# lambdaclass/ethrex

Measured on NVIDIA H100. Metric: bn254_g1_msm_points_per_sec, higher is better.
Workload: dtype u32x8 Montgomery (254-bit modular integer)

## Files before the change

ethrex_b200/csrc/msm.cu:

```cuda
#include "common.cuh"
#include "tma.cuh"
#include <cstdlib>

namespace b200zk {

static constexpr int kMaxWindows = 64;
static constexpr uint32_t kMaxPipelineChunks = 64;
static constexpr int kChunk = 16;
static constexpr int kG2MinBlocks = 1;

struct MsmPlan {
  uint32_t c, W, B;
  uint32_t chunk, T;
  uint32_t merged;
  uint32_t Wr;
  uint32_t table_stride;
  uint32_t adaptive;
};

uint32_t precompute_window(size_t n) {
  uint32_t lg = 0;
  while (((size_t)1 << lg) < n) ++lg;
  if (lg >= 20) return 20;
  if (lg <= 6) return 6;
// ... 16 lines not shown
  const uint32_t want_chunk = chunk_knob > 0 ? (uint32_t)chunk_knob : (uint32_t)kChunk;
  p.chunk = p.B < want_chunk ? p.B : want_chunk;
  p.T = p.B / p.chunk;
  p.merged = 0; p.Wr = p.W; p.table_stride = 0;
  static int adaptive = -1;
  if (adaptive < 0) { const char* e = getenv("B200ZK_SORT_MATCH"); adaptive = (e && *e == '1') ? 0 : 1; }
  p.adaptive = (uint32_t)adaptive;
  return p;
}

B2_D void decode_scalar(uint4 lo, uint4 hi, uint32_t flags, uint32_t s[8]) {
  if (flags & B200ZK_SCALARS_BE) {
    s[7] = __byte_perm(lo.x, 0, 0x0123); s[6] = __byte_perm(lo.y, 0, 0x0123); s[5] = __byte_perm(lo.z, 0, 0x0123); s[4] = __byte_perm(lo.w, 0, 0x0123);
    s[3] = __byte_perm(hi.x, 0, 0x0123); s[2] = __byte_perm(hi.y, 0, 0x0123); s[1] = __byte_perm(hi.z, 0, 0x0123); s[0] = __byte_perm(hi.w, 0, 0x0123);
  } else {
    s[0] = lo.x; s[1] = lo.y; s[2] = lo.z; s[3] = lo.w; s[4] = hi.x; s[5] = hi.y; s[6] = hi.z; s[7] = hi.w;
  }
  Fr f;
#pragma unroll
  for (int k = 0; k < 8; ++k) f.v[k] = s[k];
  if (flags & B200ZK_SCALARS_RAW) {
  } else if (flags & B200ZK_SCALARS_MONT) {
#pragma unroll 1
    for (int k = 0; k < 5; ++k) {
      Fr m = Fr::modulus(), t; uint32_t borrow = detail::sub8(t.v, f.v, m.v);
      if (!borrow) f = t;
    }
    f = Fr::from_mont(f);
  } else if (f.v[7] >= FrCfg::mod(7)) {
#pragma unroll 1
    for (int k = 0; k < 5; ++k) {
      Fr m = Fr::modulus(), t; uint32_t borrow = detail::sub8(t.v, f.v, m.v);
      if (!borrow) f = t;
    }
  }
#pragma unroll
  for (int k = 0; k < 8; ++k) s[k] = f.v[k];
}

B2_D uint32_t window_bits(const uint32_t s[8], uint32_t w, uint32_t c) {
  uint32_t bit = w * c;
  uint32_t limb = bit >> 5, off = bit & 31;
  if (limb >= 8) return 0;
  uint64_t v = s[limb];
  if (limb + 1 < 8) v |= (uint64_t)s[limb + 1] << 32;
  return (uint32_t)(v >> off) & ((1u << c) - 1u);
}

static constexpr uint32_t kNoDigit = 0xffffffffu;

static constexpr uint32_t kSkewLanes = 3;
B2_D uint32_t warp_group(uint32_t key, bool active, uint32_t* rank, uint32_t* group_mask, bool adaptive) {
  if (adaptive) {
    const uint32_t full = __activemask();
    const uint32_t act = __ballot_sync(full, active);
    const uint32_t k0 = __shfl_sync(full, key, act ? __ffs(act) - 1 : 0);
    const uint32_t m0 = __ballot_sync(full, active && key == k0);
    if (__popc(m0) < kSkewLanes) {
      *rank = 0;
      *group_mask = 1u << (threadIdx.x & 31);
      return 1;
    }
  }
  uint32_t mask = __match_any_sync(__activemask(), active ? key : kNoDigit);
  uint32_t lane = threadIdx.x & 31;
  *rank = __popc(mask & ((1u << lane) - 1u));
  *group_mask = mask;
  return __popc(mask);
}

static constexpr uint32_t kHistTile = 256;
__global__ void __launch_bounds__(kHistTile) msm_hist(const void* scalars, size_t n, uint32_t flags, MsmPlan pl, uint32_t* hist, uint32_t* digits) {
  __shared__ __align__(128) uint4 tile[2][kHistTile * 2];
  __shared__ uint64_t bar[2];
  const size_t tiles = (n + kHistTile - 1) / kHistTile;
  if (threadIdx.x == 0) { tma::barrier_init(&bar[0], 1); tma::barrier_init(&bar[1], 1); tma::barrier_init_fence(); }
  __syncthreads();
  auto issue = [&](size_t tl, uint32_t buf) {
    size_t first = tl * kHistTile;
    uint32_t bytes = (uint32_t)((n - first < kHistTile ? n - first : kHistTile) * 32);
    tma::barrier_expect(&bar[buf], bytes);
    tma::bulk_load(tile[buf], reinterpret_cast<const uint8_t*>(scalars) + first * 32, bytes, &bar[buf]);
  };
  if (threadIdx.x == 0 && blockIdx.x < tiles) issue(blockIdx.x, 0);
  uint32_t it = 0;
  for (size_t tl = blockIdx.x; tl < tiles; tl += gridDim.x, ++it) {
    const uint32_t buf = it & 1;
    if (threadIdx.x == 0 && tl + gridDim.x < tiles) issue(tl + gridDim.x, buf ^ 1);
    tma::barrier_wait(&bar[buf], (it >> 1) & 1);
    const size_t i = tl * kHistTile + threadIdx.x;
    const bool live = i < n;
    uint32_t s[8] = {0, 0, 0, 0, 0, 0, 0, 0};
    if (live) decode_scalar(tile[buf][2 * threadIdx.x], tile[buf][2 * threadIdx.x + 1], flags, s);
    uint32_t carry = 0;
    for (uint32_t w = 0; w < pl.W; ++w) {
      uint32_t coef = window_bits(s, w, pl.c) + carry;
      carry = 0;
      uint32_t neg = 0, mag = coef;
      if (w + 1 < pl.W && coef >= pl.B) { carry = 1; neg = 0x80000000u; mag = (1u << pl.c) - coef; }
      uint32_t code = mag ? ((mag - 1) | neg) : kNoDigit;
      if (live) digits[(size_t)w * n + i] = code;
      uint32_t rank, gm;
      uint32_t cnt = warp_group(mag - 1, live && mag != 0, &rank, &gm, pl.adaptive != 0);
      if (live && mag && rank == 0) atomicAdd(&hist[(pl.merged ? 0 : (size_t)w * pl.B) + (mag - 1)], cnt);
    }
    __syncthreads();
  }
}

static constexpr int kScatterIlp = 4;
__global__ void __launch_bounds__(256) msm_scatter(const uint32_t* __restrict__ digits, size_t n, MsmPlan pl, uint32_t* cursor, uint32_t* idx) {
  const size_t total = (size_t)pl.W * n;
  const size_t stride = (size_t)gridDim.x * blockDim.x;
  const size_t total_pad = (total + 31) & ~(size_t)31;
  for (size_t t0 = blockIdx.x * (size_t)blockDim.x + threadIdx.x; t0 < total_pad; t0 += stride * kScatterIlp) {
    uint32_t code[kScatterIlp], g[kScatterIlp], rank[kScatterIlp], mask[kScatterIlp], base[kScatterIlp];
    size_t w[kScatterIlp];
    bool live[kScatterIlp], active[kScatterIlp];
#pragma unroll
    for (int u = 0; u < kScatterIlp; ++u) {
      const size_t t = t0 + u * stride;
      live[u] = t < total_pad;
      code[u] = (live[u] && t < total) ? __ldg(digits + t) : kNoDigit;
      active[u] = code[u] != kNoDigit;
      w[u] = live[u] ? t / n : 0;
      g[u] = (pl.merged ? 0u : (uint32_t)(w[u] * pl.B)) + (code[u] & 0x7fffffffu);
    }
#pragma unroll
    for (int u = 0; u < kScatterIlp; ++u) {
      base[u] = 0; rank[u] = 0; mask[u] = 0;
      if (live[u]) {
        uint32_t cnt = warp_group(g[u], active[u], &rank[u], &mask[u], pl.adaptive != 0);
        if (active[u] && rank[u] == 0) base[u] = atomicAdd(&cursor[g[u]], cnt);
      }
    }
#pragma unroll
    for (int u = 0; u < kScatterIlp; ++u) {
      if (live[u]) {
        uint32_t bs = __shfl_sync(mask[u], base[u], __ffs(mask[u]) - 1);
        const size_t t = t0 + u * stride;
        if (active[u]) idx[bs + rank[u]] = (uint32_t)((t - w[u] * n) + (pl.merged ? w[u] * pl.table_stride : 0)) | (code[u] & 0x80000000u);
      }
    }
  }
}

static constexpr uint32_t kSortTile = 1024;
static constexpr uint32_t kSortMaxW = 16;
static constexpr uint32_t kSortMaxBins = 1024;
static constexpr uint32_t kSortMaxFine = 2048;
static constexpr uint32_t kSortCountSub = 4;
static constexpr int kFineIlp = 8;

struct SortPlan {
  uint32_t fb;
  uint32_t C;
  uint32_t NC;
  uint32_t range;
  uint32_t G;
};
static bool make_sort_plan(size_t n, const MsmPlan& pl, int sm_count, SortPlan* sp) {
  const size_t G = (size_t)pl.Wr * pl.B;
  uint32_t kb = 0;
  while (((size_t)1 << kb) < G) ++kb;
  if (pl.W > kSortMaxW || kb < 12 || n < ((size_t)1 << 16)) return false;
  uint32_t cb = kb > 19 ? 10 : 9;
  if (kb - cb > 11) return false;
  sp->fb = kb - cb;
  sp->C = (uint32_t)((G + ((size_t)1 << sp->fb) - 1) >> sp->fb);
  sp->G = (uint32_t)G;
  uint32_t nc = (uint32_t)sm_count;
  size_t tiles = (n + kSortTile - 1) / kSortTile;
  if (nc > tiles) nc = (uint32_t)tiles;
  size_t per = ((tiles + nc - 1) / nc) * kSortTile;
  sp->NC = (uint32_t)((n + per - 1) / per);
  sp->range = (uint32_t)per;
  return true;
}

B2_D void recode_scalar(const uint32_t s[8], const MsmPlan& pl, uint32_t (&code)[kSortMaxW]) {
  uint32_t carry = 0;
#pragma unroll
  for (uint32_t w = 0; w < kSortMaxW; ++w) {
    code[w] = kNoDigit;
    if (w < pl.W) {
      uint32_t coef = window_bits(s, w, pl.c) + carry;
      carry = 0;
      uint32_t neg = 0, mag = coef;
      if (w + 1 < pl.W && coef >= pl.B) { carry = 1; neg = 0x80000000u; mag = (1u << pl.c) - coef; }
      code[w] = mag ? ((mag - 1) | neg) : kNoDigit;
    }
  }
}

__global__ void __launch_bounds__(kHistTile) msm_sort_count(const void* scalars, size_t n, uint32_t flags, MsmPlan pl, SortPlan sp, uint32_t* cnt) {
  __shared__ __align__(128) uint4 tile[2][kHistTile * 2];
  __shared__ uint64_t bar[2];
  __shared__ uint32_t sh[kSortMaxBins];
  const uint32_t r = blockIdx.x / kSortCountSub, sub = blockIdx.x % kSortCountSub;
  for (uint32_t b = threadIdx.x; b < sp.C; b += kHistTile) sh[b] = 0;
  const size_t lo = (size_t)r * sp.range, hi = lo + sp.range < n ? lo + sp.range : n;
  const size_t tiles_all = lo < hi ? (hi - lo + kHistTile - 1) / kHistTile : 0;
  const size_t per = (tiles_all + kSortCountSub - 1) / kSortCountSub;
  const size_t t0 = sub * per, t1 = t0 + per < tiles_all ? t0 + per : tiles_all;
  if (threadIdx.x == 0) { tma::barrier_init(&bar[0], 1); tma::barrier_init(&bar[1], 1); tma::barrier_init_fence(); }
  __syncthreads();
  auto issue = [&](size_t tl, uint32_t buf) {
    size_t first = lo + tl * kHistTile;
    uint32_t bytes = (uint32_t)((hi - first < kHistTile ? hi - first : kHistTile) * 32);
    tma::barrier_expect(&bar[buf], bytes);
    tma::bulk_load(tile[buf], reinterpret_cast<const uint8_t*>(scalars) + first * 32, bytes, &bar[buf]);
  };
  if (threadIdx.x == 0 && t0 < t1) issue(t0, 0);
  uint32_t it = 0;
  for (size_t tl = t0; tl < t1; ++tl, ++it) {
    const uint32_t buf = it & 1;
    if (threadIdx.x == 0 && tl + 1 < t1) issue(tl + 1, buf ^ 1);
    tma::barrier_wait(&bar[buf], (it >> 1) & 1);
    const size_t i = lo + tl * kHistTile + threadIdx.x;
    if (i < hi) {
      uint32_t s[8], code[kSortMaxW];
      decode_scalar(tile[buf][2 * threadIdx.x], tile[buf][2 * threadIdx.x + 1], flags, s);
      recode_scalar(s, pl, code);
#pragma unroll
      for (uint32_t w = 0; w < kSortMaxW; ++w)
        if (code[w] != kNoDigit) {
          const uint32_t g = (pl.merged ? 0u : w * pl.B) + (code[w] & 0x7fffffffu);
          atomicAdd(&sh[g >> sp.fb], 1u);
        }
    }
    __syncthreads();
  }
  __syncthreads();
  for (uint32_t b = threadIdx.x; b < sp.C; b += kHistTile) if (sh[b]) atomicAdd(&cnt[(size_t)b * sp.NC + r], sh[b]);
}

struct SortCoarseSmem {
  uint2 ent[kSortTile * kSortMaxW];
  uint32_t dst[kSortTile * kSortMaxW];
  uint32_t run_base[kSortMaxBins], tile_cnt[kSortMaxBins], tile_start[kSortMaxBins];
  uint32_t warp_tot[kSortTile / 32];
  uint32_t total;
};
__global__ void __launch_bounds__(kSortTile, 1) msm_sort_coarse(const void* __restrict__ scalars, size_t n, uint32_t flags, MsmPlan pl, SortPlan sp, const uint32_t* __restrict__ base,
                                                               uint2* __restrict__ ent1) {
  extern __shared__ __align__(16) uint8_t smem_raw[];
  SortCoarseSmem& sm = *reinterpret_cast<SortCoarseSmem*>(smem_raw);
  const uint32_t r = blockIdx.x, tid = threadIdx.x;
  const size_t lo = (size_t)r * sp.range, hi = lo + sp.range < n ? lo + sp.range : n;
  const uint32_t fmask = (1u << sp.fb) - 1u;
  for (uint32_t b = tid; b < sp.C; b += kSortTile) { sm.run_base[b] = __ldg(base + (size_t)b * sp.NC + r); sm.tile_cnt[b] = 0; }
  __syncthreads();
  const uint4* sc = reinterpret_cast<const uint4*>(scalars);
  for (size_t t0 = lo; t0 < hi; t0 += kSortTile) {
    const size_t i = t0 + tid;
    uint32_t code[kSortMaxW], rank[kSortMaxW];
    const bool live = i < hi;
#pragma unroll
    for (uint32_t w = 0; w < kSortMaxW; ++w) { code[w] = kNoDigit; rank[w] = 0; }
    if (live) {
      uint32_t s[8];
      decode_scalar(__ldg(sc + 2 * i), __ldg(sc + 2 * i + 1), flags, s);
      recode_scalar(s, pl, code);
#pragma unroll
      for (uint32_t w = 0; w < kSortMaxW; ++w)
        if (code[w] != kNoDigit) {
          const uint32_t g = (pl.merged ? 0u : w * pl.B) + (code[w] & 0x7fffffffu);
          rank[w] = atomicAdd(&sm.tile_cnt[g >> sp.fb], 1u);
        }
    }
    __syncthreads();
    {
      const uint32_t v = tid < sp.C ? sm.tile_cnt[tid] : 0;
      uint32_t incl = v;
#pragma unroll
      for (int o = 1; o < 32; o <<= 1) { uint32_t t = __shfl_up_sync(0xffffffffu, incl, o); if ((tid & 31) >= (unsigned)o) incl += t; }
      if ((tid & 31) == 31) sm.warp_tot[tid >> 5] = incl;
      __syncthreads();
      uint32_t wb = 0;
      for (uint32_t k = 0; k < (tid >> 5); ++k) wb += sm.warp_tot[k];
      if (tid < sp.C) sm.tile_start[tid] = wb + incl - v;
      if (tid == kSortTile - 1) sm.total = wb + incl;
    }
    __syncthreads();
    if (live) {
#pragma unroll
      for (uint32_t w = 0; w < kSortMaxW; ++w)
        if (code[w] != kNoDigit) {
          const uint32_t g = (pl.merged ? 0u : w * pl.B) + (code[w] & 0x7fffffffu);
          const uint32_t b = g >> sp.fb, pos = sm.tile_start[b] + rank[w];
          sm.ent[pos] = make_uint2((uint32_t)(i + (pl.merged ? (size_t)w * pl.table_stride : 0)) | (code[w] & 0x80000000u), g & fmask);
          sm.dst[pos] = sm.run_base[b] + rank[w];
        }
    }
    __syncthreads();
    const uint32_t total = sm.total;
    for (uint32_t t = tid; t < total; t += kSortTile) ent1[sm.dst[t]] = sm.ent[t];
    __syncthreads();
    if (tid < sp.C) { sm.run_base[tid] += sm.tile_cnt[tid]; sm.tile_cnt[tid] = 0; }
    __syncthreads();
  }
}

static constexpr uint32_t kFineTile = 8192;
static constexpr uint32_t kFineSeg = 4 * kFineTile;
struct SortFineSmem {
  uint32_t val[kFineTile], dst[kFineTile];
  uint32_t cur[kSortMaxFine], tcnt[kSortMaxFine], tstart[kSortMaxFine];
  uint32_t warp_tot[32];
  uint32_t total;
};
B2_D void scan_fine_keys(const uint32_t* in, uint32_t* out, uint32_t F, uint32_t* warp_tot, uint32_t* total) {
  const uint32_t tid = threadIdx.x, k0 = 2 * tid, k1 = 2 * tid + 1;
  const uint32_t v0 = k0 < F ? in[k0] : 0, v1 = k1 < F ? in[k1] : 0;
  uint32_t incl = v0 + v1;
#pragma unroll
  for (int o = 1; o < 32; o <<= 1) { uint32_t t = __shfl_up_sync(0xffffffffu, incl, o); if ((tid & 31) >= (unsigned)o) incl += t; }
  if ((tid & 31) == 31) warp_tot[tid >> 5] = incl;
  __syncthreads();
  uint32_t wb = 0;
  for (uint32_t k = 0; k < (tid >> 5); ++k) wb += warp_tot[k];
  const uint32_t ex = wb + incl - v0 - v1;
  if (k0 < F) out[k0] = ex;
  if (k1 < F) out[k1] = ex + v0;
  if (tid == 1023) *total = wb + incl;
  __syncthreads();
}
__global__ void __launch_bounds__(1024) msm_sort_items(const uint32_t* __restrict__ base, SortPlan sp, uint32_t* __restrict__ item_start) {
  __shared__ uint32_t wt[32];
  const uint32_t tid = threadIdx.x;
  uint32_t v = 0;
  if (tid < sp.C) { const uint32_t sz = __ldg(base + (size_t)(tid + 1) * sp.NC) - __ldg(base + (size_t)tid * sp.NC); v = (sz + kFineSeg - 1) / kFineSeg; }
  uint32_t incl = v;
#pragma unroll
  for (int o = 1; o < 32; o <<= 1) { uint32_t t = __shfl_up_sync(0xffffffffu, incl, o); if ((tid & 31) >= (unsigned)o) incl += t; }
  if ((tid & 31) == 31) wt[tid >> 5] = incl;
  __syncthreads();
  uint32_t wb = 0;
  for (uint32_t k = 0; k < (tid >> 5); ++k) wb += wt[k];
  if (tid < sp.C) item_start[tid] = wb + incl - v;
  if (tid == sp.C - 1) item_start[sp.C] = wb + incl;
}
B2_D uint32_t item_bin(const uint32_t* __restrict__ item_start, uint32_t C, uint32_t i) {
  uint32_t lo = 0, hi = C;
  while (hi - lo > 1) { uint32_t mid = (lo + hi) >> 1; if (__ldg(item_start + mid) <= i) lo = mid; else hi = mid; }
  return lo;
}
__global__ void __launch_bounds__(1024, 2) msm_sort_fine_count(const uint2* __restrict__ ent1, SortPlan sp, const uint32_t* __restrict__ base, const uint32_t* __restrict__ item_start,
                                                               uint32_t* __restrict__ cnt2) {
  __shared__ uint32_t fh[kSortMaxFine];
  const uint32_t i = blockIdx.x, tid = threadIdx.x, F = 1u << sp.fb;
  if (i >= __ldg(item_start + sp.C)) return;
  const uint32_t b = item_bin(item_start, sp.C, i);
  const uint32_t bs = __ldg(base + (size_t)b * sp.NC), be = __ldg(base + (size_t)(b + 1) * sp.NC);
  const uint32_t s0 = bs + (i - __ldg(item_start + b)) * kFineSeg, s1 = (be - s0 > kFineSeg) ? s0 + kFineSeg : be;
  for (uint32_t k = tid; k < F; k += 1024) fh[k] = 0;
  __syncthreads();
  for (uint32_t e0 = s0 + tid; e0 < s1; e0 += 1024 * kFineIlp) {
    uint32_t kk[kFineIlp];
#pragma unroll
    for (int u = 0; u < kFineIlp; ++u) { const uint32_t e = e0 + u * 1024; kk[u] = e < s1 ? __ldg(&ent1[e].y) : 0xffffffffu; }
#pragma unroll
    for (int u = 0; u < kFineIlp; ++u) if (kk[u] != 0xffffffffu) atomicAdd(&fh[kk[u]], 1u);
  }
  __syncthreads();
  for (uint32_t k = tid; k < F; k += 1024) cnt2[(size_t)i * F + k] = fh[k];
}
__global__ void __launch_bounds__(256) msm_sort_fine_prefix(SortPlan sp, const uint32_t* __restrict__ item_start, uint32_t* __restrict__ cnt2, uint32_t* __restrict__ hist) {
  const uint32_t F = 1u << sp.fb;
  const size_t t = blockIdx.x * (size_t)blockDim.x + threadIdx.x;
  if (t >= (size_t)sp.C * F) return;
  const uint32_t b = (uint32_t)(t >> sp.fb), k = (uint32_t)t & (F - 1);
  const uint32_t i0 = __ldg(item_start + b), i1 = __ldg(item_start + b + 1);
  uint32_t run = 0;
  for (uint32_t i = i0; i < i1; ++i) {
    const size_t at = (size_t)i * F + k;
    const uint32_t c = cnt2[at];
    cnt2[at] = run;
    run += c;
  }
  if (t < sp.G) hist[t] = run;
}
__global__ void __launch_bounds__(1024, 1) msm_sort_fine_place(const uint2* __restrict__ ent1, SortPlan sp, const uint32_t* __restrict__ base, const uint32_t* __restrict__ item_start,
                                                               const uint32_t* __restrict__ cnt2, const uint32_t* __restrict__ offsets, uint32_t* __restrict__ idx) {
  extern __shared__ __align__(16) uint8_t smem_raw[];
  SortFineSmem& sm = *reinterpret_cast<SortFineSmem*>(smem_raw);
  const uint32_t i = blockIdx.x, tid = threadIdx.x, F = 1u << sp.fb;
  if (i >= __ldg(item_start + sp.C)) return;
  const uint32_t b = item_bin(item_start, sp.C, i);
  const uint32_t bs = __ldg(base + (size_t)b * sp.NC), be = __ldg(base + (size_t)(b + 1) * sp.NC);
  const uint32_t s0 = bs + (i - __ldg(item_start + b)) * kFineSeg, s1 = (be - s0 > kFineSeg) ? s0 + kFineSeg : be;
  for (uint32_t k = tid; k < F; k += 1024) {
    const size_t g = (size_t)b * F + k;
    sm.cur[k] = (g < sp.G ? __ldg(offsets + g) : 0u) + __ldg(cnt2 + (size_t)i * F + k);
    sm.tcnt[k] = 0;
  }
  __syncthreads();
  for (uint32_t t0 = s0; t0 < s1; t0 += kFineTile) {
    uint2 ev[kFineTile / 1024];
    uint32_t rank[kFineTile / 1024];
#pragma unroll
    for (int u = 0; u < (int)(kFineTile / 1024); ++u) {
      const uint32_t e = t0 + u * 1024 + tid;
      ev[u] = e < s1 ? __ldg(ent1 + e) : make_uint2(0u, 0xffffffffu);
    }
#pragma unroll
    for (int u = 0; u < (int)(kFineTile / 1024); ++u) rank[u] = ev[u].y != 0xffffffffu ? atomicAdd(&sm.tcnt[ev[u].y], 1u) : 0u;
    __syncthreads();
    scan_fine_keys(sm.tcnt, sm.tstart, F, sm.warp_tot, &sm.total);
#pragma unroll
    for (int u = 0; u < (int)(kFineTile / 1024); ++u)
      if (ev[u].y != 0xffffffffu) {
        const uint32_t pos = sm.tstart[ev[u].y] + rank[u];
        sm.val[pos] = ev[u].x;
        sm.dst[pos] = sm.cur[ev[u].y] + rank[u];
      }
    __syncthreads();
    const uint32_t total = sm.total;
    for (uint32_t t = tid; t < total; t += 1024) idx[sm.dst[t]] = sm.val[t];
    __syncthreads();
    for (uint32_t k = tid; k < F; k += 1024) { sm.cur[k] += sm.tcnt[k]; sm.tcnt[k] = 0; }
    __syncthreads();
  }
}

static constexpr int kScanThreads = 256, kScanItems = 8, kScanTile = kScanThreads * kScanItems;

B2_D uint32_t scan_value(const uint32_t* in, const uint32_t* aux, size_t i, uint32_t seg, uint32_t shift) {
  uint32_t v = in[i];
  if (!seg) return (v + (1u << shift) - 1u) >> shift;
  return (v != 0 && (aux[i] % seg) != 0) ? 1u : 0u;
}

__global__ void __launch_bounds__(kScanThreads) scan_tile_sums(const uint32_t* in, const uint32_t* aux, size_t G, uint32_t seg, uint32_t shift, uint32_t* tile_sums) {
  __shared__ uint32_t red[kScanThreads / 32];
  size_t base = (size_t)blockIdx.x * kScanTile + (size_t)threadIdx.x * kScanItems;
  uint32_t s = 0;
#pragma unroll
  for (int k = 0; k < kScanItems; ++k) if (base + k < G) s += scan_value(in, aux, base + k, seg, shift);
#pragma unroll
  for (int o = 16; o; o >>= 1) s += __shfl_xor_sync(0xffffffffu, s, o);
  if ((threadIdx.x & 31) == 0) red[threadIdx.x >> 5] = s;
  __syncthreads();
  if (threadIdx.x == 0) {
    uint32_t t = 0;
    for (int k = 0; k < kScanThreads / 32; ++k) t += red[k];
    tile_sums[blockIdx.x] = t;
  }
}
__global__ void __launch_bounds__(1024) scan_tile_offsets(uint32_t* tile_sums, size_t tiles) {
  __shared__ uint32_t buf[1024];
  __shared__ uint32_t carry;
  if (threadIdx.x == 0) carry = 0;
  __syncthreads();
  for (size_t base = 0; base < tiles; base += 1024) {
    size_t i = base + threadIdx.x;
    uint32_t v = i < tiles ? tile_sums[i] : 0;
    buf[threadIdx.x] = v;
    __syncthreads();
    for (int o = 1; o < 1024; o <<= 1) {
      uint32_t t = threadIdx.x >= (unsigned)o ? buf[threadIdx.x - o] : 0;
      __syncthreads();
      buf[threadIdx.x] += t;
      __syncthreads();
    }
    uint32_t incl = buf[threadIdx.x], c0 = carry;
    __syncthreads();
    if (i < tiles) tile_sums[i] = c0 + incl - v;
    if (threadIdx.x == 1023) carry = c0 + incl;
    __syncthreads();
  }
}
__global__ void __launch_bounds__(kScanThreads) scan_apply(const uint32_t* in, const uint32_t* aux, size_t G, uint32_t seg, uint32_t shift, const uint32_t* tile_offsets, uint32_t* offsets, uint32_t* cursor) {
  __shared__ uint32_t warp_tot[kScanThreads / 32];
  size_t base = (size_t)blockIdx.x * kScanTile + (size_t)threadIdx.x * kScanItems;
  uint32_t v[kScanItems], s = 0;
#pragma unroll
  for (int k = 0; k < kScanItems; ++k) { v[k] = base + k < G ? scan_value(in, aux, base + k, seg, shift) : 0; s += v[k]; }
  uint32_t incl = s;
#pragma unroll
  for (int o = 1; o < 32; o <<= 1) { uint32_t t = __shfl_up_sync(0xffffffffu, incl, o); if ((threadIdx.x & 31) >= (unsigned)o) incl += t; }
  if ((threadIdx.x & 31) == 31) warp_tot[threadIdx.x >> 5] = incl;
  __syncthreads();
  uint32_t wbase = 0;
  for (unsigned k = 0; k < (threadIdx.x >> 5); ++k) wbase += warp_tot[k];
  uint32_t run = tile_offsets[blockIdx.x] + wbase + incl - s;
#pragma unroll
  for (int k = 0; k < kScanItems; ++k) {
    if (base + k < G) { offsets[base + k] = seg ? run + (aux[base + k] + seg - 1) / seg : run; if (cursor) cursor[base + k] = run; }
    run += v[k];
  }
  if (blockIdx.x == gridDim.x - 1 && threadIdx.x == kScanThreads - 1) offsets[G] = seg ? run + (aux[G] + seg - 1) / seg : run;
}

static constexpr uint32_t kSegLenMax = 256;
static constexpr uint32_t kTreeRadix = 64;
static constexpr uint32_t kDirectRuns = 4;

static uint32_t pick_slice_len(size_t M, size_t resident) {
  if (M == 0) return kSegLenMax;
  size_t per_thread = (M + resident - 1) / resident;
  size_t waves = (per_thread + kSegLenMax - 1) / kSegLenMax;
  size_t len = (M + resident * waves - 1) / (resident * waves);
  if (len < 16) len = 16;
  if (len > kSegLenMax) len = kSegLenMax;
  return (uint32_t)len;
}

B2_D uint32_t bucket_of(const uint32_t* __restrict__ offsets, uint32_t G, uint32_t lo, uint32_t e) {
  uint32_t step = 1, hi = lo + 1;
  while (hi < G && __ldg(offsets + hi) <= e) { lo = hi; step <<= 1; hi = lo + step; }
  if (hi > G) hi = G;
  while (hi - lo > 1) {
    uint32_t mid = (lo + hi) >> 1;
    if (__ldg(offsets + mid) <= e) lo = mid; else hi = mid;
  }
  return lo;
}

template <class F, bool DIRECT, int MINB = 1>
__global__ void __launch_bounds__(128, MINB) msm_accumulate(const void* __restrict__ points, const uint32_t* __restrict__ idx,
                                                      const uint32_t* __restrict__ offsets, const uint32_t* __restrict__ run_off,
                                                      uint32_t G, uint32_t kSegLen, void* __restrict__ partials, uint32_t* __restrict__ run_bucket) {
  const uint32_t t = blockIdx.x * blockDim.x + threadIdx.x;
  const uint32_t M = __ldg(offsets + G);
  const uint64_t e0_64 = (uint64_t)t * kSegLen;
  if (e0_64 >= M) return;
  const uint32_t e0 = (uint32_t)e0_64;
  const uint32_t e1 = (M - e0 > kSegLen) ? e0 + kSegLen : M;
  uint32_t g;
  {
    uint32_t lo = 0, hi = G;
    while (hi - lo > 1) { uint32_t mid = (lo + hi) >> 1; if (__ldg(offsets + mid) <= e0) lo = mid; else hi = mid; }
    g = lo;
  }
  const uint32_t off0 = __ldg(offsets + g);
  uint32_t slot = t + (__ldg(run_off + g) - (off0 + kSegLen - 1) / kSegLen) + ((off0 % kSegLen) ? 1u : 0u);
  uint32_t next = __ldg(offsets + g + 1);
  XYZZ<F> acc = XYZZ<F>::identity();
  uint32_t v = DIRECT ? e0 : __ldg(idx + e0);
  Affine<F> p = load_affine_nc<F>(points, v & 0x7fffffffu);
  for (uint32_t e = e0; e < e1; ++e) {
    uint32_t vn = v; Affine<F> pn = p;
    if (e + 1 < e1) { vn = DIRECT ? e + 1 : __ldg(idx + e + 1); pn = load_affine_nc<F>(points, vn & 0x7fffffffu); }
    if (e == next) {
      store_xyzz(partials, slot, acc);
      run_bucket[slot] = g;
      ++slot;
      acc = XYZZ<F>::identity();
      g = bucket_of(offsets, G, g + 1, e);
      next = __ldg(offsets + g + 1);
    }
    if (!DIRECT && (v >> 31)) p.y = F::neg(p.y);
    xyzz_add_mixed(acc, p.x, p.y);
    v = vn; p = pn;
  }
  store_xyzz(partials, slot, acc);
  run_bucket[slot] = g;
}

__device__ __noinline__ Fq fq_mul_call(Fq a, Fq b) { return Fq::mul(a, b); }
__device__ __noinline__ Fq fq_mul2_add_call(Fq a, Fq b, Fq c, Fq d) { return Fq::mul2_add(a, b, c, d); }
__device__ __noinline__ Fq fq_mul4_add_call(Fq a, Fq b, Fq c, Fq d, Fq e, Fq f, Fq g, Fq h) { return Fq::mul4_add(a, b, c, d, e, f, g, h); }

struct PairLane {
  uint32_t mask;
  bool hi;
  B2_D Fq partner(const Fq& a) const {
    Fq r;
#pragma unroll
    for (int i = 0; i < 8; ++i) r.v[i] = __shfl_xor_sync(mask, a.v[i], 1);
    return r;
  }
  B2_D bool both(bool mine) const { return __shfl_xor_sync(mask, mine ? 1u : 0u, 1) != 0 && mine; }
  B2_D Fq sel(const Fq& if_hi, const Fq& if_lo) const {
    Fq r;
#pragma unroll
    for (int i = 0; i < 8; ++i) r.v[i] = hi ? if_hi.v[i] : if_lo.v[i];
    return r;
  }
  B2_D Fq mul(const Fq& a, const Fq& pa, const Fq& b, const Fq& pb) const {
    return fq_mul2_add_call(a, sel(pb, b), sel(pa, Fq::neg(pa)), sel(b, pb));
  }
  B2_D Fq sqr(const Fq& a, const Fq& pa) const {
    return fq_mul_call(sel(Fq::dbl(a), Fq::add(a, pa)), sel(pa, Fq::sub(a, pa)));
  }
  B2_D Fq mul2_sub(const Fq& a, const Fq& pa, const Fq& b, const Fq& pb, const Fq& c, const Fq& pc, const Fq& d, const Fq& pd) const {
    const Fq nc = Fq::neg(c);
    return fq_mul4_add_call(sel(pa, a), b, sel(a, Fq::neg(pa)), pb, sel(Fq::neg(pc), nc), d, sel(nc, pc), pd);
  }
  B2_D Fq one() const { return hi ? Fq::zero() : Fq::one(); }
};
struct XYZZHalf { Fq x, y, zz, zzz; };

B2_D void pair_mdbl(const PairLane& L, XYZZHalf& acc, const Fq& x1, const Fq& y1) {
  const Fq U = Fq::dbl(y1), pU = L.partner(U);
  const Fq V = L.sqr(U, pU), pV = L.partner(V);
  const Fq W = L.mul(U, pU, V, pV), pW = L.partner(W);
  const Fq px1 = L.partner(x1), py1 = L.partner(y1);
  const Fq S = L.mul(x1, px1, V, pV);
  const Fq xx = L.sqr(x1, px1), M = Fq::add(Fq::dbl(xx), xx), pM = L.partner(M);
  acc.x = Fq::sub(L.sqr(M, pM), Fq::dbl(S));
  const Fq T = Fq::sub(S, acc.x), pT = L.partner(T);
  acc.y = L.mul2_sub(M, pM, T, pT, W, pW, y1, py1);
  acc.zz = V; acc.zzz = W;
}
B2_D void pair_add_mixed(const PairLane& L, XYZZHalf& acc, const Fq& x2, const Fq& y2) {
  if (L.both(x2.is_zero() && y2.is_zero())) return;
  if (L.both(acc.zz.is_zero())) { acc.x = x2; acc.y = y2; acc.zz = L.one(); acc.zzz = L.one(); return; }
  const Fq pzz = L.partner(acc.zz), pzzz = L.partner(acc.zzz);
  const Fq U2 = L.mul(x2, L.partner(x2), acc.zz, pzz), S2 = L.mul(y2, L.partner(y2), acc.zzz, pzzz);
  const Fq P = Fq::sub(U2, acc.x), R = Fq::sub(S2, acc.y);
  if (L.both(P.is_zero())) {
    if (L.both(R.is_zero())) pair_mdbl(L, acc, x2, y2);
    else { acc.x = Fq::zero(); acc.y = Fq::zero(); acc.zz = Fq::zero(); acc.zzz = Fq::zero(); }
    return;
  }
  const Fq pP = L.partner(P);
  const Fq PP = L.sqr(P, pP), pPP = L.partner(PP);
  const Fq PPP = L.mul(P, pP, PP, pPP), pPPP = L.partner(PPP);
  const Fq Q = L.mul(acc.x, L.partner(acc.x), PP, pPP);
  const Fq pR = L.partner(R);
  const Fq x3 = Fq::sub(Fq::sub(L.sqr(R, pR), PPP), Fq::dbl(Q));
  const Fq T = Fq::sub(Q, x3), pT = L.partner(T);
  acc.y = L.mul2_sub(R, pR, T, pT, acc.y, L.partner(acc.y), PPP, pPPP);
  acc.x = x3;
  acc.zz = L.mul(acc.zz, pzz, PP, pPP);
  acc.zzz = L.mul(acc.zzz, pzzz, PPP, pPPP);
}

template <int MINB>
__global__ void __launch_bounds__(128, MINB) msm_accumulate_g2_pair(const void* __restrict__ points, const uint32_t* __restrict__ idx, const uint32_t* __restrict__ offsets,
                                                                const uint32_t* __restrict__ run_off, uint32_t G, uint32_t kSegLen, void* __restrict__ partials,
                                                                uint32_t* __restrict__ run_bucket) {
  const uint32_t gt = blockIdx.x * blockDim.x + threadIdx.x;
  const uint32_t t = gt >> 1;
  PairLane L;
  L.hi = (threadIdx.x & 1) != 0;
  L.mask = 3u << (threadIdx.x & 30);
  const uint32_t M = __ldg(offsets + G);
  const uint64_t e0_64 = (uint64_t)t * kSegLen;
  if (e0_64 >= M) return;
  const uint32_t e0 = (uint32_t)e0_64;
  const uint32_t e1 = (M - e0 > kSegLen) ? e0 + kSegLen : M;
  uint32_t g;
  {
    uint32_t lo = 0, hi = G;
    while (hi - lo > 1) { uint32_t mid = (lo + hi) >> 1; if (__ldg(offsets + mid) <= e0) lo = mid; else hi = mid; }
    g = lo;
  }
  const uint32_t off0 = __ldg(offsets + g);
  uint32_t slot = t + (__ldg(run_off + g) - (off0 + kSegLen - 1) / kSegLen) + ((off0 % kSegLen) ? 1u : 0u);
  uint32_t next = __ldg(offsets + g + 1);
  const uint32_t comp = L.hi ? 1u : 0u;
  auto load_half = [&](uint32_t v, Fq& x, Fq& y) {
    const size_t w = 4 * (size_t)(v & 0x7fffffffu) + comp;
    x = load_fe_nc<Fq>(points, w);
    y = load_fe_nc<Fq>(points, w + 2);
  };
  auto store_half = [&](uint32_t s, const XYZZHalf& a) {
    const size_t w = 8 * (size_t)s + comp;
    store_fe<Fq>(partials, w, a.x); store_fe<Fq>(partials, w + 2, a.y); store_fe<Fq>(partials, w + 4, a.zz); store_fe<Fq>(partials, w + 6, a.zzz);
  };
  XYZZHalf acc = {Fq::zero(), Fq::zero(), Fq::zero(), Fq::zero()};
  auto prefetch_half = [&](uint32_t v) {
    const uint8_t* q = reinterpret_cast<const uint8_t*>(points) + (4 * (size_t)(v & 0x7fffffffu) + comp) * 32;
    asm volatile("prefetch.global.L2 [%0];" ::"l"(q));
    asm volatile("prefetch.global.L2 [%0];" ::"l"(q + 64));
  };
  uint32_t v = __ldg(idx + e0);
  prefetch_half(v);
  for (uint32_t e = e0; e < e1; ++e) {
    uint32_t vn = v;
    if (e + 1 < e1) { vn = __ldg(idx + e + 1); prefetch_half(vn); }
    if (e == next) {
      store_half(slot, acc);
      if (!L.hi) run_bucket[slot] = g;
      ++slot;
      acc = {Fq::zero(), Fq::zero(), Fq::zero(), Fq::zero()};
      g = bucket_of(offsets, G, g + 1, e);
      next = __ldg(offsets + g + 1);
    }
    Fq px, py;
    load_half(v, px, py);
    if (v >> 31) py = Fq::neg(py);
    pair_add_mixed(L, acc, px, py);
    v = vn;
  }
  store_half(slot, acc);
  if (!L.hi) run_bucket[slot] = g;
}

static constexpr uint32_t kPairBatch = 256;

template <class F, bool INDIRECT>
B2_D Affine<F> pair_load(const void* __restrict__ points, const uint32_t* __restrict__ idx, uint32_t e) {
  if (INDIRECT) {
    uint32_t v = __ldg(idx + e);
    Affine<F> p = load_affine_nc<F>(points, v & 0x7fffffffu);
    if (v >> 31) p.y = F::neg(p.y);
    return p;
  }
  return load_affine_nc<F>(points, e);
}
template <class F> B2_D F pair_denominator(const Affine<F>& a, const Affine<F>& b, int* kind) {
  if (b.is_inf()) { *kind = 2; return F::one(); }
  if (a.is_inf()) { *kind = 3; return F::one(); }
  F dx = F::sub(b.x, a.x);
  if (!dx.is_zero()) { *kind = 0; return dx; }
  if (a.y == b.y && !a.y.is_zero()) { *kind = 1; return F::dbl(a.y); }
  *kind = 4; return F::one();
}

template <class F, bool INDIRECT>
B2_D void pair_load_x(const void* __restrict__ points, const uint32_t* __restrict__ idx, uint32_t e, F* x, uint32_t* v) {
  *v = INDIRECT ? __ldg(idx + e) : e;
  *x = load_field_nc(points, 2 * (size_t)(*v & 0x7fffffffu), (const F*)nullptr);
}
template <class F, bool INDIRECT>
B2_D F pair_load_y(const void* __restrict__ points, uint32_t v) {
  F y = load_field_nc(points, 2 * (size_t)(v & 0x7fffffffu) + 1, (const F*)nullptr);
  if (INDIRECT && (v >> 31)) y = F::neg(y);
  return y;
}

// ... 811 lines not shown
```

Measured before the change: 402.9 million.

## Restructure fine sort placement: larger tiles, register-held cursors, compact key staging

Reworks the fine-bucket placement kernel of the MSM sort. It doubles the tile size and halves the segments per block, and keeps per-key cursors in registers rather than shared memory. It packs the atomic rank into the key word and stores a 16-bit key plus a per-key destination base in place of a per-entry destination array, which cuts shared memory traffic and removes one barrier per tile. The scan becomes a general block scan with a warp-level scan of the warp totals instead of a serial loop over them. The packed layout assumes keys fit in 12 bits and ranks in the upper bits, which could break for larger fine widths.

```diff
diff --git a/ethrex_b200/csrc/msm.cu b/ethrex_b200/csrc/msm.cu
--- a/ethrex_b200/csrc/msm.cu
+++ b/ethrex_b200/csrc/msm.cu
@@ -342,29 +342,36 @@
   }
 }
 
-static constexpr uint32_t kFineTile = 8192;
-static constexpr uint32_t kFineSeg = 4 * kFineTile;
+static constexpr uint32_t kFineTile = 16384;
+static constexpr uint32_t kFineSeg = 2 * kFineTile;
+static constexpr uint32_t kFinePer = kFineTile / 1024, kFineKeysPerThread = kSortMaxFine / 1024;
 struct SortFineSmem {
-  uint32_t val[kFineTile], dst[kFineTile];
-  uint32_t cur[kSortMaxFine], tcnt[kSortMaxFine], tstart[kSortMaxFine];
+  uint32_t val[kFineTile];
+  uint16_t key[kFineTile];
+  uint32_t tcnt[kSortMaxFine], tstart[kSortMaxFine];
+  uint32_t dst_base[kSortMaxFine];
   uint32_t warp_tot[32];
-  uint32_t total;
 };
-B2_D void scan_fine_keys(const uint32_t* in, uint32_t* out, uint32_t F, uint32_t* warp_tot, uint32_t* total) {
-  const uint32_t tid = threadIdx.x, k0 = 2 * tid, k1 = 2 * tid + 1;
-  const uint32_t v0 = k0 < F ? in[k0] : 0, v1 = k1 < F ? in[k1] : 0;
-  uint32_t incl = v0 + v1;
-#pragma unroll
-  for (int o = 1; o < 32; o <<= 1) { uint32_t t = __shfl_up_sync(0xffffffffu, incl, o); if ((tid & 31) >= (unsigned)o) incl += t; }
-  if ((tid & 31) == 31) warp_tot[tid >> 5] = incl;
+template <uint32_t kThreads, uint32_t kPer>
+B2_D uint32_t block_scan(const uint32_t (&v)[kPer], uint32_t (&ex)[kPer], uint32_t* warp_tot) {
+  static_assert(kThreads % 32 == 0 && kThreads <= 1024, "one warp scans the warp totals");
+  const uint32_t lane = threadIdx.x & 31, warp = threadIdx.x >> 5;
+  uint32_t s = 0;
+#pragma unroll
+  for (uint32_t j = 0; j < kPer; ++j) s += v[j];
+  uint32_t incl = s;
+#pragma unroll
+  for (int o = 1; o < 32; o <<= 1) { uint32_t t = __shfl_up_sync(0xffffffffu, incl, o); if (lane >= (unsigned)o) incl += t; }
+  if (lane == 31) warp_tot[warp] = incl;
   __syncthreads();
-  uint32_t wb = 0;
-  for (uint32_t k = 0; k < (tid >> 5); ++k) wb += warp_tot[k];
-  const uint32_t ex = wb + incl - v0 - v1;
-  if (k0 < F) out[k0] = ex;
-  if (k1 < F) out[k1] = ex + v0;
-  if (tid == 1023) *total = wb + incl;
-  __syncthreads();
+  uint32_t wt = lane < kThreads / 32 ? warp_tot[lane] : 0;
+#pragma unroll
+  for (int o = 1; o < 32; o <<= 1) { uint32_t t = __shfl_up_sync(0xffffffffu, wt, o); if (lane >= (unsigned)o) wt += t; }
+  const uint32_t below = __shfl_sync(0xffffffffu, wt, (warp + 31) & 31), total = __shfl_sync(0xffffffffu, wt, 31);
+  uint32_t run = (warp ? below : 0u) + incl - s;
+#pragma unroll
+  for (uint32_t j = 0; j < kPer; ++j) { ex[j] = run; run += v[j]; }
+  return total;
 }
 __global__ void __launch_bounds__(1024) msm_sort_items(const uint32_t* __restrict__ base, SortPlan sp, uint32_t* __restrict__ item_start) {
   __shared__ uint32_t wt[32];
@@ -425,42 +432,54 @@
                                                                const uint32_t* __restrict__ cnt2, const uint32_t* __restrict__ offsets, uint32_t* __restrict__ idx) {
   extern __shared__ __align__(16) uint8_t smem_raw[];
   SortFineSmem& sm = *reinterpret_cast<SortFineSmem*>(smem_raw);
+  constexpr uint32_t kNoKey = 0xfffu;
   const uint32_t i = blockIdx.x, tid = threadIdx.x, F = 1u << sp.fb;
   if (i >= __ldg(item_start + sp.C)) return;
   const uint32_t b = item_bin(item_start, sp.C, i);
   const uint32_t bs = __ldg(base + (size_t)b * sp.NC), be = __ldg(base + (size_t)(b + 1) * sp.NC);
   const uint32_t s0 = bs + (i - __ldg(item_start + b)) * kFineSeg, s1 = (be - s0 > kFineSeg) ? s0 + kFineSeg : be;
-  for (uint32_t k = tid; k < F; k += 1024) {
+  uint32_t cur[kFineKeysPerThread];
+#pragma unroll
+  for (uint32_t j = 0; j < kFineKeysPerThread; ++j) {
+    const uint32_t k = tid * kFineKeysPerThread + j;
     const size_t g = (size_t)b * F + k;
-    sm.cur[k] = (g < sp.G ? __ldg(offsets + g) : 0u) + __ldg(cnt2 + (size_t)i * F + k);
+    cur[j] = k < F ? (g < sp.G ? __ldg(offsets + g) : 0u) + __ldg(cnt2 + (size_t)i * F + k) : 0u;
     sm.tcnt[k] = 0;
   }
   __syncthreads();
   for (uint32_t t0 = s0; t0 < s1; t0 += kFineTile) {
-    uint2 ev[kFineTile / 1024];
-    uint32_t rank[kFineTile / 1024];
-#pragma unroll
-    for (int u = 0; u < (int)(kFineTile / 1024); ++u) {
+    uint32_t val[kFinePer], kr[kFinePer];
+#pragma unroll
+    for (uint32_t u = 0; u < kFinePer; ++u) {
       const uint32_t e = t0 + u * 1024 + tid;
-      ev[u] = e < s1 ? __ldg(ent1 + e) : make_uint2(0u, 0xffffffffu);
-    }
-#pragma unroll
-    for (int u = 0; u < (int)(kFineTile / 1024); ++u) rank[u] = ev[u].y != 0xffffffffu ? atomicAdd(&sm.tcnt[ev[u].y], 1u) : 0u;
+      kr[u] = kNoKey; val[u] = 0;
+      if (e < s1) { const uint2 x = __ldg(ent1 + e); val[u] = x.x; kr[u] = x.y; }
+    }
+#pragma unroll
+    for (uint32_t u = 0; u < kFinePer; ++u) if (kr[u] != kNoKey) kr[u] |= atomicAdd(&sm.tcnt[kr[u]], 1u) << 12;
     __syncthreads();
-    scan_fine_keys(sm.tcnt, sm.tstart, F, sm.warp_tot, &sm.total);
-#pragma unroll
-    for (int u = 0; u < (int)(kFineTile / 1024); ++u)
-      if (ev[u].y != 0xffffffffu) {
-        const uint32_t pos = sm.tstart[ev[u].y] + rank[u];
-        sm.val[pos] = ev[u].x;
-        sm.dst[pos] = sm.cur[ev[u].y] + rank[u];
+    uint32_t v[kFineKeysPerThread], ex[kFineKeysPerThread];
+#pragma unroll
+    for (uint32_t j = 0; j < kFineKeysPerThread; ++j) v[j] = sm.tcnt[tid * kFineKeysPerThread + j];
+    const uint32_t total = block_scan<1024, kFineKeysPerThread>(v, ex, sm.warp_tot);
+#pragma unroll
+    for (uint32_t j = 0; j < kFineKeysPerThread; ++j) {
+      const uint32_t k = tid * kFineKeysPerThread + j;
+      sm.tstart[k] = ex[j];
+      sm.dst_base[k] = cur[j] - ex[j];
+      cur[j] += v[j];
+      sm.tcnt[k] = 0;
+    }
+    __syncthreads();
+#pragma unroll
+    for (uint32_t u = 0; u < kFinePer; ++u)
+      if (kr[u] != kNoKey) {
+        const uint32_t k = kr[u] & kNoKey, pos = sm.tstart[k] + (kr[u] >> 12);
+        sm.val[pos] = val[u];
+        sm.key[pos] = (uint16_t)k;
       }
     __syncthreads();
-    const uint32_t total = sm.total;
-    for (uint32_t t = tid; t < total; t += 1024) idx[sm.dst[t]] = sm.val[t];
-    __syncthreads();
-    for (uint32_t k = tid; k < F; k += 1024) { sm.cur[k] += sm.tcnt[k]; sm.tcnt[k] = 0; }
-    __syncthreads();
+    for (uint32_t t = tid; t < total; t += 1024) idx[sm.dst_base[sm.key[t]] + t] = sm.val[t];
   }
 }
 
```

After: 411.8 million (median of 6 runs). +2.2%, better.
